# AdityaNG/SOccDPT

Measured on AMD Instinct MI355X. Metric: frames/sec SOccDPT_V3 swin2_tiny_256 @256px (depth+seg+points+occupancy forward), higher is better.
Workload: dtype mixed fp16 + f16x3 (SOCCDPT_PREC_MIXED: fp16 MFMA operands, x3 split per the shipped precision map; f32 accumulate)

## Files before the change

### soccdpt_amd/csrc/capi.cpp

```cpp
#include <hip/hip_runtime.h>

#include <cstring>
#include <cstdlib>
#include <string>

#include "internal.h"
#include "calibrate.h"
#include "train.h"
#include "kernels.h"
#include "occ_eval.h"
#include "visualise.h"
#include "occ_view.h"
#include "batch_targets.h"
#include "../../include/soccdpt_vis.h"
#include "../../include/soccdpt_occ_view.h"
#include "../../include/soccdpt_data.h"

using namespace soccdpt;

static std::string g_create_error;

namespace soccdpt {
LaunchTimer*& launch_timer() {
    static thread_local LaunchTimer* t = nullptr;
    return t;
}
unsigned long long& launch_counter() {
    static thread_local unsigned long long n = 0;
    return n;
}
void set_last_error(const std::string& msg) { g_create_error = msg; }
}

static double occ_cells(const soccdpt_config& c) { return (double)c.grid[0] * c.grid[1] * c.grid[2] * c.num_classes; }

static int fail(Handle* h, const std::string& msg) {
    if (h) h->err = msg; else g_create_error = msg;
    return 1;
}

static int profiled_project(Handle* h, const float* inv, const float* seg, int B, int in_h, int in_w, float* inv_up, float* seg_up, float* points,
                            uint32_t* occ_bits, int clear_bits, hipStream_t st) {
    const soccdpt_config& c = h->cfg;
    const double px = (double)c.cam_width * c.cam_height * B;
    const double bytes = (double)B * in_h * in_w * 4.0 * (1 + c.num_classes) + px * 4.0 * ((inv_up ? 1 : 0) + (seg_up ? c.num_classes : 0) + (points ? 3 : 0));
    ProfScope ps(h->prof, "project_voxelise", 0.0, bytes, st);
    return launch_project(c, inv, seg, B, in_h, in_w, inv_up, seg_up, points, occ_bits, clear_bits, st, h->err);
}
static int profiled_occ_expand(Handle* h, const uint32_t* bits, int B, float* occ, hipStream_t st) {
// ... 308 lines not shown
}

int soccdpt_occ_expand(void* handle, const uint32_t* dev_bits, int B, float* dev_occ, void* stream) {
    Handle* h = static_cast<Handle*>(handle);
    if (!h) return 1;
    if (B <= 0) return fail(h, "soccdpt_occ_expand: empty batch");
    return profiled_occ_expand(h, dev_bits, B, dev_occ, (hipStream_t)stream);
}

int soccdpt_occ_zero(void* handle, int B, float* dev_occ, void* stream) {
    Handle* h = static_cast<Handle*>(handle);
    if (!h) return 1;
    if (B <= 0 || !dev_occ) return fail(h, "soccdpt_occ_zero: bad argument");
    ProfScope ps(h->prof, "occ_zero", 0.0, occ_cells(h->cfg) * 4.0 * B, (hipStream_t)stream);
    return launch_occ_zero(h->cfg, B, dev_occ, (hipStream_t)stream, h->err);
}

int soccdpt_occ_set(void* handle, const uint32_t* dev_bits, int B, float* dev_occ, void* stream) {
    Handle* h = static_cast<Handle*>(handle);
    if (!h) return 1;
    if (B <= 0 || !dev_occ || !dev_bits) return fail(h, "soccdpt_occ_set: bad argument");
    ProfScope ps(h->prof, "occ_set", 0.0, occ_cells(h->cfg) * 0.125, (hipStream_t)stream);
    return launch_occ_set(h->cfg, dev_bits, B, dev_occ, (hipStream_t)stream, h->err);
}

int soccdpt_forward(void* handle, const float* dev_x, int B, float* dev_inv_up, float* dev_seg_up, float* dev_points,
                    float* dev_occ, uint32_t* dev_occ_bits, void* dev_workspace, size_t workspace_bytes, void* stream) {
    Handle* h = static_cast<Handle*>(handle);
    if (!h) return 1;
    if (B <= 0) return fail(h, "soccdpt_forward: empty batch");
    const int S = h->img;
    hipStream_t st = (hipStream_t)stream;
    float *inv, *seg;
    int rc = network_at_head(h, "soccdpt_forward", dev_x, B, dev_workspace, workspace_bytes, st, &inv, &seg);
    if (rc) return rc;
    const bool occ_on = h->cfg.compute_occ != 0;
    if (occ_on && !dev_occ_bits) return fail(h, "soccdpt_forward: compute_occ needs dev_occ_bits");
    rc = profiled_project(h, inv, seg, B, S, S, dev_inv_up, dev_seg_up, dev_points, occ_on ? dev_occ_bits : nullptr, 1, st);
    if (rc) return rc;
    if (occ_on && dev_occ) rc = profiled_occ_expand(h, dev_occ_bits, B, dev_occ, st);
    return rc;
}

int soccdpt_voxelise_frames(void* handle, const float* dev_inv_up, const float* dev_seg, int B, int in_h, int in_w, uint32_t* dev_frame_bits,
                            int clear_bits, void* stream) {
    Handle* h = static_cast<Handle*>(handle);
    if (!h) return 1;
    if (!dev_inv_up || !dev_seg || !dev_frame_bits) return fail(h, "soccdpt_voxelise_frames: null argument");
    if (B <= 0 || in_h <= 0 || in_w <= 0) return fail(h, "soccdpt_voxelise_frames: empty input");
    return profiled_voxelise_frames(h, dev_inv_up, dev_seg, B, in_h, in_w, dev_frame_bits, clear_bits, (hipStream_t)stream);
}

int soccdpt_occ_expand_frames(void* handle, const uint32_t* dev_frame_bits, int B, float* dev_occ, void* stream) {
    Handle* h = static_cast<Handle*>(handle);
    if (!h) return 1;
    if (!dev_frame_bits || !dev_occ) return fail(h, "soccdpt_occ_expand_frames: null argument");
    if (B <= 0) return fail(h, "soccdpt_occ_expand_frames: empty batch");
    return profiled_occ_expand_frames(h, dev_frame_bits, B, dev_occ, (hipStream_t)stream);
}

int soccdpt_forward_frames(void* handle, const float* dev_x, int B, float* dev_inv_up, float* dev_seg_up, float* dev_points, float* dev_occ,
                           uint32_t* dev_occ_bits, uint32_t* dev_frame_bits, void* dev_workspace, size_t workspace_bytes, void* stream) {
    Handle* h = static_cast<Handle*>(handle);
    if (!h) return 1;
    if (B <= 0) return fail(h, "soccdpt_forward_frames: empty batch");
    if (!dev_x || !dev_workspace) return fail(h, "soccdpt_forward_frames: null argument");
    if (!h->cfg.compute_occ) return fail(h, "soccdpt_forward_frames: the handle was created without compute_occ");
    if (!dev_inv_up) return fail(h, "soccdpt_forward_frames: dev_inv_up is required (the per-frame voxelisation reads the inverse depth back)");
    if (!dev_frame_bits) return fail(h, "soccdpt_forward_frames: dev_frame_bits is required");
    const int S = h->img;
    hipStream_t st = (hipStream_t)stream;
// ... 271 lines not shown
    if (d.x3 && d.tune == 12 && d.splitk <= 1 && !d.ln_g &&
        (d.stride != 1 || d.pad != 1 || d.in_halo != 1 || d.Hi || d.Wi || d.gather1 || d.grp_rows || d.seg2_k || d.stamps))
        return fail(nullptr, "soccdpt_op_igemm: x3 configuration 12 has no generalised addressing");
    if (launch_igemm(d, (hipStream_t)stream, err)) return fail(nullptr, err);
    if (a->gn_stats && a->gn_count && (gn_bm <= 0 || a->gn_hw % gn_bm))
        return fail(nullptr, "soccdpt_op_igemm: statistics requested but the chosen tile has no statistics epilogue (tune forces a tile without one)");
    if (a->gn_stats && a->gn_count && launch_gn_finish(a->gn_part, a->gn_stats, a->M / a->gn_hw, a->gn_hw / gn_bm, a->N / a->gn_cpg, a->gn_hw, a->gn_cpg, 1e-5f, (hipStream_t)stream, err))
        return fail(nullptr, err);
    return 0;
}

int soccdpt_op_depth_tail(const void* dev_d1, const void* dev_wt, const float* dev_bias, const float* dev_w4, float b4, float* dev_out, int precision,
                          int B, int h, int w, void* stream) {
    std::string err;
    if (!dev_d1 || !dev_wt || !dev_bias || !dev_w4 || !dev_out) return fail(nullptr, "soccdpt_op_depth_tail: null argument");
    if (precision != SOCCDPT_PREC_BF16 && precision != SOCCDPT_PREC_F16) return fail(nullptr, "soccdpt_op_depth_tail: precision is SOCCDPT_PREC_BF16 or _F16");
    if (B <= 0 || h <= 0 || w <= 0) return fail(nullptr, "soccdpt_op_depth_tail: B, h, w must be positive");
    if ((2 * h) % 8 || (2 * w) % 16) return fail(nullptr, "soccdpt_op_depth_tail: the output (2h x 2w) must be a multiple of 8 x 16");
    if (launch_depth_tail(static_cast<const bf16_t*>(dev_d1), static_cast<const bf16_t*>(dev_wt), dev_bias, dev_w4, b4, dev_out, precision == SOCCDPT_PREC_F16 ? 1 : 0,
                          B, h, w, (hipStream_t)stream, err))
        return fail(nullptr, err);
    return 0;
}

int soccdpt_op_seg_tail(const float* dev_part, int nplanes, const float* dev_bias, float* dev_tmp, float* dev_out, int B, int h, int w, int sigmoid,
                        void* stream) {
    std::string err;
    if (!dev_part || !dev_bias || !dev_tmp || !dev_out) return fail(nullptr, "soccdpt_op_seg_tail: null argument");
    if (nplanes < 1 || B <= 0 || h <= 0 || w <= 0) return fail(nullptr, "soccdpt_op_seg_tail: nplanes, B, h and w must be positive");
    if (launch_seg_tail_parts(dev_part, nplanes, dev_bias, dev_tmp, dev_out, B, h, w, sigmoid ? 1 : 0, (hipStream_t)stream, err)) return fail(nullptr, err);
    return 0;
}

int soccdpt_op_wgrad_tn(const void* dev_a, long lda, const void* dev_b, long ldb, size_t K, int Nout, int C, int taps, int rp, int precision, float* dev_scratch,
                        size_t scratch_floats, float* dev_out, void* stream) {
    std::string err;
    if (!dev_a || !dev_b || !dev_scratch || !dev_out) return fail(nullptr, "soccdpt_op_wgrad_tn: null argument");
    if (precision != SOCCDPT_PREC_BF16 && precision != SOCCDPT_PREC_F16 && precision != SOCCDPT_PREC_F16X3) return fail(nullptr, "soccdpt_op_wgrad_tn: bf16, fp16 or f16x3 operands");
    const OpFmt fmt = precision == SOCCDPT_PREC_F16X3 ? OpFmt::X3 : (precision == SOCCDPT_PREC_F16 ? OpFmt::F16 : OpFmt::BF16);
    if (tr_wgrad_tn(dev_a, lda, dev_b, ldb, K, Nout, C, taps, rp, fmt, dev_scratch, scratch_floats, dev_out,
                    (hipStream_t)stream, err))
        return fail(nullptr, err);
    return 0;
}

size_t soccdpt_op_train_layer_bwd_scratch_bytes(const soccdpt_train_layer_bwd_args* args) {
    std::string err;
    const size_t n = args ? train_layer_bwd_scratch_bytes(*args, err) : 0;
    if (!n) fail(nullptr, args ? err : "soccdpt_op_train_layer_bwd_scratch_bytes: null args");
    return n;
}
int soccdpt_op_train_layer_bwd(void* handle, const soccdpt_train_layer_bwd_args* args, void* dev_scratch, size_t scratch_bytes, uint32_t* path_out, void* stream) {
    Handle* h = static_cast<Handle*>(handle);
    if (!h) return fail(nullptr, "soccdpt_op_train_layer_bwd: null handle");
    if (!args) return fail(h, "soccdpt_op_train_layer_bwd: null args");
    unsigned path = 0;
    if (train_layer_bwd(*h, *args, dev_scratch, scratch_bytes, &path, (hipStream_t)stream, h->err)) return 1;
    if (path_out) *path_out = path;
    return 0;
}

size_t soccdpt_op_train_aux_scratch_bytes(const soccdpt_train_aux_args* args) {
    std::string err;
    const size_t n = args ? train_aux_scratch_bytes(*args, err) : 0;
    if (!n) fail(nullptr, args ? err : "soccdpt_op_train_aux_scratch_bytes: null args");
    return n;
// ... 302 lines not shown
```

### soccdpt_amd/csrc/elementwise.hip

```cpp
#include <type_traits>

#include "half16.h"
#include "kernels.h"
#include "ln_body.h"

namespace soccdpt {

__device__ __forceinline__ float row_sum(float v) {
    auto ror = [](float x, auto n) {
        return __builtin_bit_cast(float, __builtin_amdgcn_update_dpp(0, __builtin_bit_cast(int, x), 0x120 + decltype(n)::value, 0xf, 0xf, true));
    };
    v += ror(v, std::integral_constant<int, 8>{});
    v += ror(v, std::integral_constant<int, 4>{});
    v += ror(v, std::integral_constant<int, 2>{});
    v += ror(v, std::integral_constant<int, 1>{});
    return v;
}

#define LAUNCH_HF(hf, K, ...)                                   \
    do {                                                        \
        if (hf) SOCCDPT_LAUNCH((K<true>), __VA_ARGS__);     \
        else SOCCDPT_LAUNCH((K<false>), __VA_ARGS__);       \
    } while (0)

// ... 428 lines not shown
    for (size_t i = (size_t)blockIdx.x * blockDim.x + threadIdx.x; i < total; i += (size_t)gridDim.x * blockDim.x) {
        const int ox = (int)(i % W);
        size_t r = i / W;
        const int oy = (int)(r % H), b = (int)(r / H);
        const float fy = sy * (float)oy, fx = sx * (float)ox;
        const int y0 = (int)fy, x0 = (int)fx;
        const int y1 = y0 + (y0 < h - 1), x1 = x0 + (x0 < w - 1);
        const float ly = fy - (float)y0, lx = fx - (float)x0, hy = 1.f - ly, hx = 1.f - lx;
        const float* base = in + (size_t)b * h * w * 3;
#pragma unroll
        for (int c = 0; c < 3; ++c) {
            const float v = hy * (hx * base[((size_t)y0 * w + x0) * 3 + c] + lx * base[((size_t)y0 * w + x1) * 3 + c]) +
                            ly * (hx * base[((size_t)y1 * w + x0) * 3 + c] + lx * base[((size_t)y1 * w + x1) * 3 + c]);
            const float a = sigmoid ? 1.f / (1.f + expf(-v)) : 0.5f * tanhf(v) + 0.5f;
            out[((size_t)(b * 3 + c) * H + oy) * W + ox] = a;
        }
    }
}

__global__ __launch_bounds__(256) void seg_logits_finish_kernel(const float* __restrict__ part , const float* __restrict__ bias, float* __restrict__ out ,
                                                                 size_t M, int T) {
    for (size_t m = (size_t)blockIdx.x * blockDim.x + threadIdx.x; m < M; m += (size_t)gridDim.x * blockDim.x) {
        float4 a = *reinterpret_cast<const float4*>(part + m * 4);
        for (int t = 1; t < T; ++t) {
            const float4 v = *reinterpret_cast<const float4*>(part + ((size_t)t * M + m) * 4);
            a.x += v.x; a.y += v.y; a.z += v.z;
        }
        out[m * 3 + 0] = a.x + bias[0];
        out[m * 3 + 1] = a.y + bias[1];
        out[m * 3 + 2] = a.z + bias[2];
    }
}

int launch_seg_tail_parts(const float* part, int ntiles, const float* bias, float* tmp, float* seg, int B, int h, int wd, int sigmoid, hipStream_t st, std::string& err) {
    const size_t M = (size_t)B * h * wd;
    size_t blocks = (M + 255) / 256;
    if (blocks > 2048) blocks = 2048;
    SOCCDPT_LAUNCH(seg_logits_finish_kernel, dim3((unsigned)blocks), dim3(256), 0, st, part, bias, tmp, M, ntiles);
    if (check_launch("seg_logits_finish", err)) return 1;
    const size_t total = (size_t)B * 4 * h * wd;
    blocks = (total + 255) / 256;
    if (blocks > 2048) blocks = 2048;
    SOCCDPT_LAUNCH(seg_up_act_kernel, dim3((unsigned)blocks), dim3(256), 0, st, tmp, seg, B, h, wd, sigmoid);
    return check_launch("seg_up_act", err);
}

int launch_seg_tail(const void* feat, int feat_is_f32, int hf, const float* w, const float* bias, float* tmp, float* seg, int B, int h, int wd,
                    int sigmoid, hipStream_t st, std::string& err, int* path) {
    if (!ptr_aligned16(feat) || (!feat_is_f32 && !ptr_aligned16(w))) { err = "seg_tail: 16-byte aligned features (and weights beside 16-bit features)"; return 1; }
    if (path) *path = feat_is_f32 ? SOCCDPT_FWD_PATH_SEG_F32 : SOCCDPT_FWD_PATH_SEG_16;
    const int M = B * h * wd;
    const dim3 grid((unsigned)(((size_t)M * 16 + 255) / 256));
    unsigned gl = grid.x > 2048 ? 2048 : grid.x;
    if (feat_is_f32) SOCCDPT_LAUNCH(conv1x1_c3_f32_kernel, grid, dim3(256), 0, st, static_cast<const float*>(feat), w, bias, tmp, M);
    else LAUNCH_HF(hf, conv1x1_c3_kernel, dim3(gl), dim3(256), 0, st, static_cast<const bf16_t*>(feat), w, bias, tmp, M);
    if (check_launch("conv1x1_c3", err)) return 1;
    const size_t total = (size_t)B * 4 * h * wd;
    size_t blocks = (total + 255) / 256;
    if (blocks > 2048) blocks = 2048;
    SOCCDPT_LAUNCH(seg_up_act_kernel, dim3((unsigned)blocks), dim3(256), 0, st, tmp, seg, B, h, wd, sigmoid);
    return check_launch("seg_up_act", err);
}

template <bool F16>
__global__ void cvt_bf16_kernel(const float* __restrict__ in, bf16_t* __restrict__ out, size_t n) {
    for (size_t i = (size_t)blockIdx.x * blockDim.x + threadIdx.x; i < n; i += (size_t)gridDim.x * blockDim.x) out[i] = f2h<F16>(in[i]);
}
// ... 144 lines not shown
```

### soccdpt_amd/csrc/internal.h

```cpp
#pragma once
#include <hip/hip_runtime.h>
#include <stdint.h>

#include <memory>
#include <string>
#include <unordered_map>
#include <vector>

#include "../../include/soccdpt_hip.h"
#include "launch.h"
#include "params.h"

namespace soccdpt {

struct Prepared;

struct ProfRec {
    const char* name;
    double flops, bytes;
    size_t first_pair, n_pairs;
};
struct Profiler : LaunchTimer {
    bool on = false;
    std::vector<ProfRec> recs;
// ... 30 lines not shown
    }
};

struct SiteRec {
    int M, N, K, taps, cfg, count;
    char name[16];
};

struct Handle {
    soccdpt_config cfg;
    int device = 0;
    int img = 256;
    Arch arch;
    std::string err;
    bool prof_sites = false;
    std::vector<SiteRec> sites;
    std::unordered_map<long long, int> tune_by_shape;
    bool fuse_qkv = true;
    int fuse_qkv_mask = 3;
    int mlp_fuse_max = 128;
    std::unordered_map<std::string, int> prec_map;
    int prec_source = -1;
    unsigned long long calib_fp = 0;
    bool calib_fp_valid = false;
    std::vector<WeightSlot> weights;
    ModelP params;
    const float* W(PRef r) const { return r.i < 0 ? nullptr : weights[r.i].ptr; }
    float* G(PRef r) const { return r.i < 0 ? nullptr : weights[r.i].grad; }
    std::unordered_map<std::string, int> index;
    size_t prepared_bytes = 0;
    Prepared* prep = nullptr;
    bool is_prepared = false;
    int launches = 0;
    Profiler prof;
    int n_streams = 1;
    std::vector<hipStream_t> sub_streams;
    std::vector<hipEvent_t> join_events;
    bool use_graph = false;
    struct GraphKey {
        const void *x = nullptr, *inv = nullptr, *seg = nullptr, *ws = nullptr;
        int B = 0, streams = 0;
        bool operator==(const GraphKey& o) const { return x == o.x && inv == o.inv && seg == o.seg && ws == o.ws && B == o.B && streams == o.streams; }
    } graph_key;
    struct WsKey {
        const void* ws = nullptr;
        int B = 0, streams = 0;
        bool operator==(const WsKey& o) const { return ws == o.ws && B == o.B && streams == o.streams; }
    } ws_key;
    int ws_zero_fills = 0;
    struct TrainKey {
        const void* ws = nullptr;
        int B = 0;
        float dropout_p = 0.f;
        int amp = 0;
        float drop_path = 0.f;
    } train_key;
    float train_drop_path = 0.f;
    std::shared_ptr<void> layer_state;
    int train_amp = 0;
    hipGraph_t graph = nullptr;
    hipGraphExec_t graph_exec = nullptr;
    hipStream_t graph_stream = nullptr;
    hipEvent_t graph_in = nullptr, graph_out = nullptr;
    int eager_calls = 0;
    ~Handle();
};

int model_init(Handle& h, std::string& err);
int model_bind(Handle& h, const char* key, const void* ptr, const int64_t* shape, int ndim, std::string& err);
size_t model_workspace_bytes(Handle& h, int B);
int model_prepare(Handle& h, void* prepared, size_t bytes, hipStream_t stream, std::string& err);
int model_network(Handle& h, const float* x, int B, float* inv256, float* seg256, void* ws, size_t ws_bytes, hipStream_t stream,
                  std::string& err);

std::vector<std::string> model_prec_groups(const Handle& h);
void model_prec_default(Handle& h);
int model_prec_set(Handle& h, const char* pattern, int fmt, std::string& err);
bool model_prec_x2w_ok(const std::string& group);
int model_set_streams(Handle& h, int n, std::string& err);
void model_drop_graph(Handle& h);
int model_workspace_tensor(Handle& h, int B, const char* name, size_t* byte_offset, size_t* elems, int* kind, int* H, int* W, int* C);

int launch_project(const soccdpt_config& cfg, const float* inv, const float* seg, int B, int in_h, int in_w, float* inv_up,
                   float* seg_up, float* points, uint32_t* occ_bits, int clear_bits, hipStream_t stream, std::string& err);
int launch_occ_expand(const soccdpt_config& cfg, const uint32_t* bits, int B, float* occ, hipStream_t stream, std::string& err);
int launch_occ_zero(const soccdpt_config& cfg, int B, float* occ, hipStream_t stream, std::string& err);
int launch_occ_set(const soccdpt_config& cfg, const uint32_t* bits, int B, float* occ, hipStream_t stream, std::string& err);
int launch_occ_or(const soccdpt_config& cfg, uint32_t* dst, const uint32_t* src, int nsets, hipStream_t stream, std::string& err);

int launch_voxelise_frames(const soccdpt_config& cfg, const float* inv_up, const float* seg, int B, int in_h, int in_w, uint32_t* frame_bits,
                           int clear_bits, hipStream_t stream, std::string& err);
int launch_occ_expand_frames(const soccdpt_config& cfg, const uint32_t* frame_bits, int B, float* occ, hipStream_t stream, std::string& err);

}
```

### soccdpt_amd/csrc/kernels.h

```cpp
#pragma once
#include <hip/hip_runtime.h>
#include <stdint.h>

#include <string>

#include "../../include/soccdpt_hip.h"
#include "igemm.h"

namespace soccdpt {

inline int check_launch(const char* what, std::string& err) {
    hipError_t e = hipGetLastError();
    if (e != hipSuccess) {
        err = std::string(what) + ": " + hipGetErrorString(e);
        return 1;
    }
    return 0;
}

inline bool ptr_aligned16(const void* p) { return reinterpret_cast<uintptr_t>(p) % 16 == 0; }

int launch_patch_embed(const float* x, const float* w, const float* bias, const float* g, const float* beta, float* xf, bf16_t* xb,
                       int hf, int B, int S, int C0, hipStream_t st, std::string& err);
int launch_ln_residual(const float* y, const float* g, const float* beta, float* xf, bf16_t* xb, bf16_t* halo, float* halo_f32, int hf, int M,
                       int C, int residual, int res, int merge, hipStream_t st, std::string& err, const float* row_scale = nullptr, int rows_per_scale = 1,
                       int hf_halo = -1, int* path = nullptr);
int launch_merge_gather(const void* in, void* out, int B, int R, int C, int elem_bytes, hipStream_t st, std::string& err);
int launch_bilinear(const void* in, int in_is_bf16, float* out_f32, bf16_t* out_bf16, float* out_f32_halo, int out_halo, int hf, int B, int h,
                    int w, int H, int W, int C, hipStream_t st, std::string& err, int* path = nullptr);
int launch_seg_tail(const void* feat, int feat_is_f32, int hf, const float* w, const float* bias, float* tmp, float* seg, int B, int h, int wd,
                    int sigmoid, hipStream_t st, std::string& err, int* path = nullptr);
int launch_seg_tail_parts(const float* part, int ntiles, const float* bias, float* tmp, float* seg, int B, int h, int wd, int sigmoid, hipStream_t st, std::string& err);
inline int patch_w_ld(int C0) { return C0 <= 128 ? 128 : 192; }
int launch_patch_w(const float* w, float* out, int C0, hipStream_t st, std::string& err);
int launch_cvt_bf16(const float* in, bf16_t* out, size_t n, int hf, hipStream_t st, std::string& err);
int launch_conv_w(const float* in, const float* scale, void* out, int out_is_f32, int hf, int Cout, int Cin, hipStream_t st, std::string& err);
int launch_bn_fold(const float* g, const float* b, const float* mean, const float* var, float* scale, float* shift, int C, hipStream_t st,
                   std::string& err);
int launch_qkv_bias(const float* q, const float* v, float* out, int C, hipStream_t st, std::string& err);
int launch_logit_scale(const float* ls, float* out, int H, hipStream_t st, std::string& err);
int launch_cpb_table(const float* w0, const float* b0, const float* w2, float* table, int ws, int pws, int H, hipStream_t st,
                     std::string& err);

int launch_depth_tail(const bf16_t* d1, const bf16_t* wt, const float* bias, const float* w4, float b4, float* out, int hf, int B, int h,
                      int w, hipStream_t st, std::string& err);

size_t metrics_scratch_bytes(int B, int C);
int launch_depth_metrics(const float* pred, const float* gt, const uint8_t* mask, int B, size_t npix, float* out, void* scratch, hipStream_t st,
                         std::string& err);
int launch_iou_metrics(const float* pred, const float* gt, int B, int C, size_t npix, float* out, void* scratch, hipStream_t st, std::string& err);

size_t loss_scratch_bytes(int B, int H, int W, int h, int w);
int launch_training_loss(int B, int H, int W, int h, int w, int C, int compute_ss, float alpha, float w_d, float w_s, const float* inv,
                         const float* seg, const float* y_disp, const uint8_t* mask_disp, const float* y_seg, const uint8_t* mask_seg,
                         float* out, float* d_inv, float* d_seg, void* scratch, hipStream_t st, std::string& err);

int launch_gt_occupancy(int B, int H, int W, int C, const double* intr, const double* pc_scale, const double* pc_shift, const double* rot27,
                        const float* occ_shape, const int* grid, float threshold, const float* disparity, const int32_t* seg_class, float* depth,
                        double* points, uint32_t* counts, uint8_t* occ, hipStream_t st, std::string& err);

size_t upsample_bwd_scratch_bytes(const soccdpt_config& cfg, int B, int h);
int launch_upsample_bwd(const soccdpt_config& cfg, const float* inv_up, const float* d_inv_up, const float* d_seg_up, const float* d_points, int B, int h, int w,
                        float* d_inv, float* d_seg, void* scratch, hipStream_t st, std::string& err);

int launch_input_transform_u8(const uint8_t* img, int B, int Hs, int Ws, int Hd, int Wd, const double* mean, const double* stdv, float* out,
// ... 85 lines not shown
```

### soccdpt_amd/csrc/model.cpp

```cpp
#include <cstdio>
#include <cstdlib>
#include <cstring>

#include <unordered_set>

#include "internal.h"
#include "kernels.h"

namespace soccdpt {

struct BlockW {
    const void *qkv_w, *proj_w, *fc1_w, *fc2_w;
    float *qkv_bias, *scale, *table, *bias_acc;
};
struct RcuW { const void *w1, *w2; };
struct RnBlockW { const void *ds_w = nullptr, *c1_w = nullptr, *c2_w = nullptr, *c3_w = nullptr; };
struct VitBlockW { const void *qkv_w, *proj_w, *fc1_w, *fc2_w; };
struct HybridW {
    const void* stem_w = nullptr;
    std::vector<RnBlockW> rn;
    const void* pe_w = nullptr;
    float* pos = nullptr;
    std::vector<VitBlockW> blocks;
    const void *ro_w[2] = {nullptr, nullptr}, *pp_w[2] = {nullptr, nullptr}, *pp4_w = nullptr;
// ... 830 lines not shown
               RUN(launch_bilinear(w.oc[0], 0, nullptr, fH == 2 ? nullptr : static_cast<bf16_t*>(w.path1), fH == 2 ? static_cast<float*>(w.path1) : nullptr, 1, fH == 2 ? 0 : fH, B, r, r,
                                   2 * r, 2 * r, F, st, err)); }
    }
    const int r1 = 2 * a.fres(0), r0 = 4 * a.fres(0);
    {
        IgemmDesc d = conv(w.path1, F, P.d0_w, F / 2, r1);
        d.bias = W(MP.depth.c0.b);
        if (fD2 <= 1 && F == 256) {
            d.out_op = w.d1; d.out_fmt = MIX ? fD2 : -1;
            RUN(gemm(d, fH));
            PROF("depth_tail_fused", 2.0 * B * r0 * r0 * 32.0 * 9.0 * (F / 2), 0.0);
            RUN(launch_depth_tail(static_cast<const bf16_t*>(w.d1), static_cast<const bf16_t*>(P.d2_w), W(MP.depth.c2.b), W(MP.depth.c4.w), P.d4_b, inv256, fD2, B, r1, r1, st, err));
        } else {
            const bool d1_16 = fH <= 1 && !MIX;
            if (d1_16) d.out_op = w.d1; else to_plain(d, w.d1, fH);
            RUN(gemm(d, fH));
            { PROF("bilinear_resize", 0.0, (double)B * r1 * r1 * (F / 2) * (2.0 + 8.0));
              RUN(launch_bilinear(w.d1, d1_16 ? 1 : 0, nullptr, fD2 == 2 ? nullptr : static_cast<bf16_t*>(w.d1u), fD2 == 2 ? static_cast<float*>(w.d1u) : nullptr, 1, fD2 == 2 ? 0 : fD2, B, r1,
                                  r1, r0, r0, F / 2, st, err)); }
            d = conv(w.d1u, F / 2, P.d2_w, 32, r0);
            d.bias = W(MP.depth.c2.b); d.act = ACT_RELU; d.dot_w = W(MP.depth.c4.w); d.dot_b = P.d4_b; d.out_dot = inv256;
            RUN(gemm(d, fD2));
        }
        const int fS1 = MIX ? GF("head.s1") : fH;
        const bool s1_f32 = fS1 >= 2;
        d = conv(w.path1, F, P.s0_w, F, r1);
        d.bias = P.bn_shift; d.act = ACT_RELU;
        if (seg_dot3_active(h)) {
            d.dot3 = 1; d.dot_w = W(MP.seg.c4.w); d.out_dot = static_cast<float*>(w.s1);
            d.f16 = fH == 1;
            const int parts = F / igemm_dot3_bn(d);
            RUN(gemm(d, fH));
            PROF("seg_tail", 0.0, (double)B * r1 * r1 * (parts * 16.0 + 12.0 + 12.0 + 48.0));
            RUN(launch_seg_tail_parts(static_cast<const float*>(w.s1), parts, W(MP.seg.c4.b), w.s2, seg256, B, r1, r1, h.cfg.sigmoid, st, err));
        } else {
        if (s1_f32) to_plain(d, w.s1, fH); else { d.out_op = w.s1; d.out_fmt = MIX ? 1 : -1; }
        RUN(gemm(d, fH));
        { PROF("seg_tail", 0.0, (double)B * r1 * r1 * (F * 2.0 + 12.0 + 48.0));
          RUN(launch_seg_tail(w.s1, s1_f32 ? 1 : 0, fS1 == 1, W(MP.seg.c4.w), W(MP.seg.c4.b), w.s2, seg256, B, r1, r1, h.cfg.sigmoid, st, err)); }
        }
        ++launches;
    }
#undef RUN
#undef PROF
    return 0;
}

static void chunk_range(int B, int n, int i, int& lo, int& hi) {
    const int base = B / n, rem = B % n;
    lo = i * base + (i < rem ? i : rem);
    hi = lo + base + (i < rem ? 1 : 0);
}

static int n_chunks(const Handle& h, int B) {
    int n = h.n_streams < 1 ? 1 : h.n_streams;
    return n > B ? B : n;
}

static void carve_all(const Handle& h, int B, Arena& ar, std::vector<Workspace>& ws) {
    ar.take<float>((size_t)B * h.img * h.img * (1 + h.cfg.num_classes));
    const int n = n_chunks(h, B);
    ws.resize(n);
    for (int i = 0; i < n; ++i) {
        int lo, hi;
        chunk_range(B, n, i, lo, hi);
        carve(h, hi - lo, ar, ws[i]);
    }
}

size_t model_workspace_bytes(Handle& h, int B) {
    Arena ar(nullptr, 0);
    std::vector<Workspace> ws;
    carve_all(h, B, ar, ws);
    return ar.off + 256;
}

int model_set_streams(Handle& h, int n, std::string& err) {
    if (n < 1 || n > 8) { err = "soccdpt_set_streams: n must be in 1..8"; return 1; }
    while ((int)h.sub_streams.size() < n - 1) {
        hipStream_t s;
        if (hipStreamCreateWithFlags(&s, hipStreamNonBlocking) != hipSuccess) { err = "soccdpt_set_streams: stream creation failed"; return 1; }
        h.sub_streams.push_back(s);
    }
    while ((int)h.join_events.size() < n) {
        hipEvent_t e;
        if (hipEventCreateWithFlags(&e, hipEventDisableTiming) != hipSuccess) { err = "soccdpt_set_streams: event creation failed"; return 1; }
        h.join_events.push_back(e);
    }
    h.n_streams = n;
    model_drop_graph(h);
    return 0;
}

static int network_eager(Handle& h, const float* x, int B, float* inv256, float* seg256, void* ws, size_t ws_bytes, hipStream_t st,
                         std::string& err) {
    Arena ar(ws, ws_bytes);
    std::vector<Workspace> wsp;
    carve_all(h, B, ar, wsp);
    if (ar.off > ws_bytes) { err = "soccdpt_network: workspace too small"; return 1; }
    const int n = (int)wsp.size();
// ... 23 lines not shown
    }
    h.launches = launches;
    return 0;
}

void model_drop_graph(Handle& h) {
    if (h.graph_exec) (void)hipGraphExecDestroy(h.graph_exec);
    if (h.graph) (void)hipGraphDestroy(h.graph);
    h.graph_exec = nullptr;
    h.graph = nullptr;
    h.eager_calls = 0;
}

int model_network(Handle& h, const float* x, int B, float* inv256, float* seg256, void* ws, size_t ws_bytes, hipStream_t st,
                  std::string& err) {
    if (!h.is_prepared) { err = "soccdpt_network: call soccdpt_prepare after binding weights"; return 1; }
    if (B <= 0 || !x || !inv256 || !seg256 || !ws) { err = "soccdpt_network: bad argument"; return 1; }
    {
        int dev = -1;
        (void)hipGetDevice(&dev);
        if (dev != h.device) { err = "soccdpt_network: the handle was created on device " + std::to_string(h.device) + " but device " + std::to_string(dev) + " is current"; return 1; }
        const size_t need = model_workspace_bytes(h, B);
        if (ws_bytes < need) { err = "soccdpt_network: workspace too small (soccdpt_workspace_bytes)"; return 1; }
        Handle::WsKey wk{ws, B, h.n_streams};
        if (!(wk == h.ws_key)) {
            model_drop_graph(h);
            if (hipMemsetAsync(ws, 0, need, st) != hipSuccess) { err = "soccdpt_network: workspace zero-fill failed"; return 1; }
            h.ws_key = wk;
            h.ws_zero_fills++;
        }
    }
    if (!h.use_graph || h.prof.on) return network_eager(h, x, B, inv256, seg256, ws, ws_bytes, st, err);
    Handle::GraphKey key;
    key.x = x; key.inv = inv256; key.seg = seg256; key.ws = ws; key.B = B; key.streams = h.n_streams;
    if (!(key == h.graph_key)) {
        model_drop_graph(h);
        h.graph_key = key;
    }
    if (h.eager_calls++ == 0 && !h.graph_exec) return network_eager(h, x, B, inv256, seg256, ws, ws_bytes, st, err);
    hipStream_t cs = h.graph_stream;
    if (hipEventRecord(h.graph_in, st) != hipSuccess || hipStreamWaitEvent(cs, h.graph_in, 0) != hipSuccess) {
        err = "soccdpt_network: graph fork failed";
        return 1;
    }
    if (!h.graph_exec) {
        if (hipStreamBeginCapture(cs, hipStreamCaptureModeThreadLocal) != hipSuccess) { err = "soccdpt_network: begin capture failed"; return 1; }
        const int rc = network_eager(h, x, B, inv256, seg256, ws, ws_bytes, cs, err);
        hipGraph_t g = nullptr;
        const hipError_t ec = hipStreamEndCapture(cs, &g);
        if (rc || ec != hipSuccess || !g) {
            if (g) (void)hipGraphDestroy(g);
            if (!rc) err = std::string("soccdpt_network: end capture failed: ") + hipGetErrorString(ec);
            return 1;
        }
        h.graph = g;
        if (hipGraphInstantiate(&h.graph_exec, g, nullptr, nullptr, 0) != hipSuccess) {
            model_drop_graph(h);
            err = "soccdpt_network: graph instantiate failed";
            return 1;
        }
    }
    if (hipGraphLaunch(h.graph_exec, cs) != hipSuccess) { err = "soccdpt_network: hipGraphLaunch failed"; return 1; }
    if (hipEventRecord(h.graph_out, cs) != hipSuccess || hipStreamWaitEvent(st, h.graph_out, 0) != hipSuccess) {
        err = "soccdpt_network: graph join failed";
        return 1;
    }
    return 0;
// ... 4 lines not shown
```

### soccdpt_amd/lib.py

```python
from __future__ import annotations

import ctypes
import os
from typing import Optional, Sequence

import numpy as np
import torch

_HERE = os.path.dirname(os.path.abspath(__file__))
LIB_PATH = os.environ.get("SOCCDPT_LIB_PATH") or os.path.join(_HERE, "libsoccdpt_hip.so")

ABI_VERSION = 12
BACKBONE_IDS = {"swin2t16_256": 0, "swin2b24_384": 1, "vitb_rn50_384": 2, "swin2l24_384": 3, "swinl12_384": 5}
PREC_BF16 = 0
PREC_F32 = 1
PREC_F16 = 2
PREC_F16X3 = 3
PREC_MIXED = 4
PREC_F16X2W = 5


class SoccdptConfig(ctypes.Structure):
    _fields_ = [
        ("abi_version", ctypes.c_int32),
# ... 258 lines not shown
        "soccdpt_pack_targets": (ci, [vp, ci, cs, vp, ci, vp, ci, vp, ci, ci, ci, ci, ci, vp, vp, vp, vp, vp]),
        "soccdpt_pack_expand": (ci, [vp, ci, cs, vp, ci, ci, ci, ci, vp, vp]),
    }


PACK_PROTOTYPES = _pack_prototypes()


def _swin1_prototypes() -> dict:
    vp, ci, cf = ctypes.c_void_p, ctypes.c_int, ctypes.c_float
    return {
        "soccdpt_swin1_window_attention": (ci, [vp, vp, vp, vp, ci, ci, ci, ci, ci, ci, ci, vp]),
        "soccdpt_swin1_ln_rows": (ci, [vp, vp, vp, vp, ci, ci, ci, cf, vp]),
        "soccdpt_swin1_merge_ln": (ci, [vp, vp, vp, vp, ci, ci, ci, ci, cf, vp]),
    }


SWIN1_PROTOTYPES = _swin1_prototypes()


def _occ_view_prototypes() -> dict:
    vp, ci, cs, cd = ctypes.c_void_p, ctypes.c_int, ctypes.c_size_t, ctypes.c_double
    i32, u8, f64 = ctypes.POINTER(ctypes.c_int32), ctypes.POINTER(ctypes.c_uint8), ctypes.POINTER(cd)
    return {
        "soccdpt_occ_view_columns": (ci, [vp, ci, i32, ci, ci, ci, vp, vp, vp, vp, vp]),
        "soccdpt_occ_view_paint": (ci, [vp, vp, ci, ci, ci, ci, ci, vp, ci, u8, ci, ci, ci, ci, ci, vp, cs, cs, cs, cs, vp]),
        "soccdpt_occ_view_iou2d": (ci, [vp, ci, vp, ci, cs, ci, vp, vp]),
        "soccdpt_occ_view_splat": (ci, [vp, ci, i32, ci, f64, f64, cd, ci, cd, ci, ci, vp, vp]),
        "soccdpt_occ_view_resolve": (ci, [vp, vp, ci, ci, ci, ci, ci, vp, ci, vp, cs, cs, cs, cs, vp]),
    }


OCC_VIEW_PROTOTYPES = _occ_view_prototypes()
PACK_INDEX_BITS = (1, 2, 4, 8)


def load_library() -> ctypes.CDLL:
    global _lib
    if _lib is not None:
        return _lib
    if not os.path.exists(LIB_PATH):
        raise RuntimeError(
            f"{LIB_PATH} is missing: build it with `python -c 'import __graft_entry__ as g; g.build()'` "
            "(make -C soccdpt_amd/csrc).  The SOccDPT MI355X path has no CPU fallback.")
    L = ctypes.CDLL(LIB_PATH)
    for table in (PROTOTYPES, VIS_PROTOTYPES, DATA_PROTOTYPES, PACK_PROTOTYPES, SWIN1_PROTOTYPES, OCC_VIEW_PROTOTYPES):
        for symbol, (restype, argtypes) in table.items():
            fn = getattr(L, symbol)
            fn.restype, fn.argtypes = restype, argtypes
    if L.soccdpt_abi_version() != ABI_VERSION:
        raise RuntimeError("libsoccdpt_hip.so ABI version mismatch; rebuild the library")
    for which, cls in ((0, SoccdptConfig), (1, IgemmArgs), (2, KernelStat), (3, CalibReport), (4, CalibOptions), (5, TrainLayerBwdArgs), (6, TrainAuxArgs), (7, FwdAuxArgs)):
        if L.soccdpt_sizeof(which) != ctypes.sizeof(cls):
            raise RuntimeError(f"libsoccdpt_hip.so: sizeof mismatch for {cls.__name__}: library {L.soccdpt_sizeof(which)}, binding {ctypes.sizeof(cls)}")
    _lib = L
    return L


def _ptr(t: Optional[torch.Tensor]) -> Optional[int]:
    if t is None:
        return None
    assert t.is_contiguous(), "device tensors handed to libsoccdpt_hip must be contiguous"
    return t.data_ptr()


def _stream_ptr(device: torch.device) -> int:
    return torch.cuda.current_stream(device).cuda_stream


def _call(symbol: str, *args, device: torch.device, guard: bool = True):
    L = load_library()
    fn = getattr(L, symbol)
    if guard:
        with torch.cuda.device(device):
            rc = fn(*args, _stream_ptr(device))
    else:
        rc = fn(*args, _stream_ptr(device))
    if rc != 0:
        raise RuntimeError(f"{symbol} failed: {L.soccdpt_last_error(None).decode()}")
# ... 352 lines not shown
def op_igemm(x, wt, M, N, Cin, taps=1, ldx=0, H=0, W=0, bias=None, res1=None, res2=None, act=0, out_f32=None,
             act_on_f32=0, out_bf16=None, out_halo=0, dot_w=None, dot_b=0.0, out_dot=None, tune=-1, f32=0, precision=None, splitk=1, sk_part=None, sk_count=None,
             conv=None, gather1=0, grp_rows=0, grp_off=0, grp_stride=0, seg2_k=0, seg2_off=0, gn_stats=None, gn_part=None, gn_count=None, gn_cpg=0, gn_hw=0,
             stamps=None, sk_defer=0, res2_h=0, res2_w=0, ln_g=None, ln_b=None, ln_xf=None, ln_halo=None, ln_residual=1, dot3=0, out_fmt=-1,
             halo_fmt=-1):
    c = conv or {}
    a = IgemmArgs(_ptr(x), _ptr(wt), M, N, Cin, taps, ldx, H, W, _ptr(bias), _ptr(res1), _ptr(res2), act, _ptr(out_f32),
                  act_on_f32, _ptr(out_bf16), out_halo, _ptr(dot_w), float(dot_b), _ptr(out_dot), tune,
                  int(precision) if precision is not None else (PREC_F32 if f32 else PREC_BF16), int(splitk), _ptr(sk_part), _ptr(sk_count),
                  0 if sk_part is None else sk_part.numel(), 0 if sk_count is None else sk_count.numel(),
                  1 if conv else 0, c.get("stride", 1), c.get("pad", 1), c.get("in_halo", 1), c.get("Hi", 0), c.get("Wi", 0), int(gather1),
                  int(grp_rows), int(grp_off), int(seg2_k), int(seg2_off), int(grp_stride),
                  _ptr(gn_stats), _ptr(gn_part), _ptr(gn_count), int(gn_cpg), int(gn_hw),
                  0 if gn_part is None else gn_part.numel(), 0 if gn_count is None else gn_count.numel(), _ptr(stamps), int(sk_defer),
                  int(res2_h), int(res2_w), _ptr(ln_g), _ptr(ln_b), _ptr(ln_xf), _ptr(ln_halo), int(ln_residual), int(dot3), int(out_fmt),
                  int(halo_fmt))
    _call("soccdpt_op_igemm", ctypes.byref(a), device=x.device, guard=False)


def op_depth_tail(d1, wt, bias, w4, b4, out, B, h, w, precision=PREC_BF16):
    _call("soccdpt_op_depth_tail", _ptr(d1), _ptr(wt), _ptr(bias), _ptr(w4), float(b4), _ptr(out), int(precision), int(B), int(h), int(w),
          device=d1.device, guard=False)


def op_seg_tail(part, nplanes, bias, tmp, out, B, h, w, sigmoid):
    _call("soccdpt_op_seg_tail", _ptr(part), int(nplanes), _ptr(bias), _ptr(tmp), _ptr(out), int(B), int(h), int(w), 1 if sigmoid else 0,
          device=part.device, guard=False)


def op_gn_finish(part, stats, B, tps, groups, hw, cpg, eps=1e-5):
    _call("soccdpt_op_gn_finish", _ptr(part), _ptr(stats), int(B), int(tps), int(groups), int(hw), int(cpg), float(eps), device=part.device, guard=False)


def op_gn_apply(raw, stats, gamma, beta, hw, w, cpg, part=None, tps=0, raw2=None, stats2=None, part2=None, tps2=0, gamma2=None, beta2=None, res=None,
                out_f32=None, out_op=None, out_halo=None, out_format=PREC_F32, relu=True, eps=1e-5):
    M, C = raw.shape
    _call("soccdpt_op_gn_apply", _ptr(raw), _ptr(stats), _ptr(part), int(tps), _ptr(gamma), _ptr(beta), _ptr(raw2), _ptr(stats2), _ptr(part2), int(tps2),
          _ptr(gamma2), _ptr(beta2), _ptr(res), _ptr(out_f32), _ptr(out_op), _ptr(out_halo), int(out_format), 1 if relu else 0, M, int(hw),
          int(w), int(C), int(cpg), float(eps), device=raw.device, guard=False)


def op_vit_attention(qkv, out, B, N, heads, precision=PREC_BF16, out_x3=False):
    if out_x3:
        _call("soccdpt_op_vit_attention_out", _ptr(qkv), _ptr(out), int(precision), 1, B, N, heads, device=qkv.device, guard=False)
    else:
        _call("soccdpt_op_vit_attention", _ptr(qkv), _ptr(out), int(precision), B, N, heads, device=qkv.device, guard=False)


def op_input_transform_u8(frames: torch.Tensor, Hd: int, Wd: int, mean=(0.5, 0.5, 0.5), std=(0.5, 0.5, 0.5)) -> torch.Tensor:
    assert frames.dtype == torch.uint8 and frames.dim() == 4 and frames.shape[3] == 3 and frames.is_cuda
    B, Hs, Ws, _ = frames.shape
    out = torch.empty((B, 3, Hd, Wd), dtype=torch.float32, device=frames.device)
    m, s = (ctypes.c_double * 3)(*mean), (ctypes.c_double * 3)(*std)
    _call("soccdpt_input_transform_u8", _ptr(frames), B, Hs, Ws, Hd, Wd, m, s, _ptr(out), device=frames.device)
    return out


_DATA_DTYPES = {torch.uint8: DATA_U8, torch.uint16: DATA_U16, torch.float32: DATA_F32}


def op_data_targets(seg: torch.Tensor, colors: torch.Tensor, disp: Optional[torch.Tensor] = None, flip: bool = False, want_onehot: bool = True,
                    want_class_map: bool = False, want_y_disp: Optional[bool] = None, want_unmatched: bool = True) -> dict:
    assert seg.is_cuda and seg.dtype == torch.uint8 and seg.dim() == 4 and seg.shape[3] == 3, "seg must be a cuda uint8 [B,H,W,3] tensor"
    assert colors.is_cuda and colors.dtype == torch.uint8 and colors.dim() == 2 and colors.shape[1] == 3, "colors must be a cuda uint8 [C,3] tensor"
    B, H, W, _ = seg.shape
    C = colors.shape[0]
# ... 174 lines not shown
```

Before: 3957.

## Fuse seg tail logits and upsample into one kernel and fold occupancy-bit clearing

Replaces the two-launch segmentation tail (logit reduction, then bilinear upsample plus activation) with a single fused kernel. The upsample recomputes the partial-logit sums per output pixel instead of reading them back from a temporary. The same kernel also zeroes the occupancy bit buffer, so the later projection step skips its own clear, removing a memset/launch. The fused path recomputes each logit four times per output pixel, and there is no grid-wide sync between writing the logits temp and the upsample reading it, but the upsample only recomputes and never reads the temp.

Measured after the change: 3973 (median of 6 runs). No clear change (+0.4%).

```diff
diff --git a/include/soccdpt_fwd_ends.h b/include/soccdpt_fwd_ends.h
--- /dev/null
+++ b/include/soccdpt_fwd_ends.h
@@ -0,0 +1,18 @@
+#ifndef SOCCDPT_FWD_ENDS_H
+#define SOCCDPT_FWD_ENDS_H
+
+#include <stddef.h>
+#include <stdint.h>
+
+#ifdef __cplusplus
+extern "C" {
+#endif
+
+int soccdpt_op_seg_tail_clear(const float* dev_part, int nplanes, const float* dev_bias, float* dev_tmp, float* dev_out, int B, int h, int w,
+                              int sigmoid, uint32_t* dev_zero, size_t nzero, void* stream);
+
+#ifdef __cplusplus
+}
+#endif
+
+#endif
diff --git a/soccdpt_amd/csrc/capi.cpp b/soccdpt_amd/csrc/capi.cpp
--- a/soccdpt_amd/csrc/capi.cpp
+++ b/soccdpt_amd/csrc/capi.cpp
@@ -15,6 +15,7 @@
 #include "../../include/soccdpt_vis.h"
 #include "../../include/soccdpt_occ_view.h"
 #include "../../include/soccdpt_data.h"
+#include "../../include/soccdpt_fwd_ends.h"
 
 using namespace soccdpt;
 
@@ -389,11 +390,16 @@
     const int S = h->img;
     hipStream_t st = (hipStream_t)stream;
     float *inv, *seg;
-    int rc = network_at_head(h, "soccdpt_forward", dev_x, B, dev_workspace, workspace_bytes, st, &inv, &seg);
-    if (rc) return rc;
     const bool occ_on = h->cfg.compute_occ != 0;
     if (occ_on && !dev_occ_bits) return fail(h, "soccdpt_forward: compute_occ needs dev_occ_bits");
-    rc = profiled_project(h, inv, seg, B, S, S, dev_inv_up, dev_seg_up, dev_points, occ_on ? dev_occ_bits : nullptr, 1, st);
+    const bool fold = occ_on && ptr_aligned16(dev_occ_bits) && model_fold_clear_ok(*h, B);
+    h->fold_bits = fold ? dev_occ_bits : nullptr;
+    h->fold_words = fold ? soccdpt_occ_words(h) : 0;
+    int rc = network_at_head(h, "soccdpt_forward", dev_x, B, dev_workspace, workspace_bytes, st, &inv, &seg);
+    h->fold_bits = nullptr;
+    h->fold_words = 0;
+    if (rc) return rc;
+    rc = profiled_project(h, inv, seg, B, S, S, dev_inv_up, dev_seg_up, dev_points, occ_on ? dev_occ_bits : nullptr, fold ? 0 : 1, st);
     if (rc) return rc;
     if (occ_on && dev_occ) rc = profiled_occ_expand(h, dev_occ_bits, B, dev_occ, st);
     return rc;
@@ -731,6 +737,16 @@
     return 0;
 }
 
+int soccdpt_op_seg_tail_clear(const float* dev_part, int nplanes, const float* dev_bias, float* dev_tmp, float* dev_out, int B, int h, int w, int sigmoid,
+                              uint32_t* dev_zero, size_t nzero, void* stream) {
+    std::string err;
+    if (!dev_part || !dev_bias || !dev_tmp || !dev_out) return fail(nullptr, "soccdpt_op_seg_tail_clear: null argument");
+    if (nplanes < 1 || B <= 0 || h <= 0 || w <= 0) return fail(nullptr, "soccdpt_op_seg_tail_clear: nplanes, B, h and w must be positive");
+    if (launch_seg_tail_parts(dev_part, nplanes, dev_bias, dev_tmp, dev_out, B, h, w, sigmoid ? 1 : 0, (hipStream_t)stream, err, dev_zero, dev_zero ? nzero : 0))
+        return fail(nullptr, "soccdpt_op_seg_tail_clear: " + err);
+    return 0;
+}
+
 int soccdpt_op_wgrad_tn(const void* dev_a, long lda, const void* dev_b, long ldb, size_t K, int Nout, int C, int taps, int rp, int precision, float* dev_scratch,
                         size_t scratch_floats, float* dev_out, void* stream) {
     std::string err;
diff --git a/soccdpt_amd/csrc/elementwise.hip b/soccdpt_amd/csrc/elementwise.hip
--- a/soccdpt_amd/csrc/elementwise.hip
+++ b/soccdpt_amd/csrc/elementwise.hip
@@ -484,7 +484,70 @@
     }
 }
 
-int launch_seg_tail_parts(const float* part, int ntiles, const float* bias, float* tmp, float* seg, int B, int h, int wd, int sigmoid, hipStream_t st, std::string& err) {
+__global__ __launch_bounds__(256) void seg_tail_fused_kernel(const float* __restrict__ part , const float* __restrict__ bias,
+                                                              float* __restrict__ logits , float* __restrict__ out , int B,
+                                                              int h, int w, int T, int sigmoid, uint32_t* __restrict__ zero, size_t nzero) {
+    const int H = 2 * h, W = 2 * w;
+    const size_t total = (size_t)B * H * W, M = (size_t)B * h * w;
+    const float sy = (float)(h - 1) / (float)(H - 1), sx = (float)(w - 1) / (float)(W - 1);
+    const float bs[3] = {bias[0], bias[1], bias[2]};
+    if (zero) {
+        const size_t n4 = nzero / 4;
+        uint4* z4 = reinterpret_cast<uint4*>(zero);
+        for (size_t i = (size_t)blockIdx.x * blockDim.x + threadIdx.x; i < n4; i += (size_t)gridDim.x * blockDim.x) z4[i] = uint4{0u, 0u, 0u, 0u};
+        for (size_t i = n4 * 4 + (size_t)blockIdx.x * blockDim.x + threadIdx.x; i < nzero; i += (size_t)gridDim.x * blockDim.x) zero[i] = 0u;
+    }
+    auto logit = [&](size_t m, float (&v)[3]) {
+        float4 a = *reinterpret_cast<const float4*>(part + m * 4);
+        for (int t = 1; t < T; ++t) {
+            const float4 p = *reinterpret_cast<const float4*>(part + ((size_t)t * M + m) * 4);
+            a.x += p.x; a.y += p.y; a.z += p.z;
+        }
+        v[0] = a.x + bs[0]; v[1] = a.y + bs[1]; v[2] = a.z + bs[2];
+    };
+    for (size_t m = (size_t)blockIdx.x * blockDim.x + threadIdx.x; m < M; m += (size_t)gridDim.x * blockDim.x) {
+        float v[3];
+        logit(m, v);
+        logits[m * 3 + 0] = v[0]; logits[m * 3 + 1] = v[1]; logits[m * 3 + 2] = v[2];
+    }
+    for (size_t i = (size_t)blockIdx.x * blockDim.x + threadIdx.x; i < total; i += (size_t)gridDim.x * blockDim.x) {
+        const int ox = (int)(i % W);
+        size_t r = i / W;
+        const int oy = (int)(r % H), b = (int)(r / H);
+        const float fy = sy * (float)oy, fx = sx * (float)ox;
+        const int y0 = (int)fy, x0 = (int)fx;
+        const int y1 = y0 + (y0 < h - 1), x1 = x0 + (x0 < w - 1);
+        const float ly = fy - (float)y0, lx = fx - (float)x0, hy = 1.f - ly, hx = 1.f - lx;
+        const size_t base = (size_t)b * h * w;
+        float v00[3], v01[3], v10[3], v11[3];
+        logit(base + (size_t)y0 * w + x0, v00); logit(base + (size_t)y0 * w + x1, v01);
+        logit(base + (size_t)y1 * w + x0, v10); logit(base + (size_t)y1 * w + x1, v11);
+#pragma unroll
+        for (int c = 0; c < 3; ++c) {
+            const float v = hy * (hx * v00[c] + lx * v01[c]) + ly * (hx * v10[c] + lx * v11[c]);
+            const float a = sigmoid ? 1.f / (1.f + expf(-v)) : 0.5f * tanhf(v) + 0.5f;
+            out[((size_t)(b * 3 + c) * H + oy) * W + ox] = a;
+        }
+    }
+}
+
+static bool seg_tail_two_launches() {
+    static const bool two = getenv("SOCCDPT_SEG_TAIL_FUSED") && atoi(getenv("SOCCDPT_SEG_TAIL_FUSED")) == 0;
+    return two;
+}
+int seg_tail_parts_launches() { return seg_tail_two_launches() ? 2 : 1; }
+
+int launch_seg_tail_parts(const float* part, int ntiles, const float* bias, float* tmp, float* seg, int B, int h, int wd, int sigmoid, hipStream_t st, std::string& err,
+                          uint32_t* zero, size_t nzero) {
+    if (!seg_tail_two_launches()) {
+        if (!ptr_aligned16(part) || !ptr_aligned16(zero)) { err = "seg_tail: 16-byte aligned partial logits (and words to clear)"; return 1; }
+        const size_t total = (size_t)B * 4 * h * wd;
+        size_t blocks = (total + 255) / 256;
+        if (blocks > 2048) blocks = 2048;
+        SOCCDPT_LAUNCH(seg_tail_fused_kernel, dim3((unsigned)blocks), dim3(256), 0, st, part, bias, tmp, seg, B, h, wd, ntiles, sigmoid, zero, nzero);
+        return check_launch("seg_tail_fused", err);
+    }
+    if (zero && hipMemsetAsync(zero, 0, nzero * sizeof(uint32_t), st) != hipSuccess) { err = "seg_tail: clearing failed"; return 1; }
     const size_t M = (size_t)B * h * wd;
     size_t blocks = (M + 255) / 256;
     if (blocks > 2048) blocks = 2048;
diff --git a/soccdpt_amd/csrc/internal.h b/soccdpt_amd/csrc/internal.h
--- a/soccdpt_amd/csrc/internal.h
+++ b/soccdpt_amd/csrc/internal.h
@@ -86,15 +86,17 @@
     Prepared* prep = nullptr;
     bool is_prepared = false;
     int launches = 0;
+    uint32_t* fold_bits = nullptr;
+    size_t fold_words = 0;
     Profiler prof;
     int n_streams = 1;
     std::vector<hipStream_t> sub_streams;
     std::vector<hipEvent_t> join_events;
     bool use_graph = false;
     struct GraphKey {
-        const void *x = nullptr, *inv = nullptr, *seg = nullptr, *ws = nullptr;
+        const void *x = nullptr, *inv = nullptr, *seg = nullptr, *ws = nullptr, *bits = nullptr;
         int B = 0, streams = 0;
-        bool operator==(const GraphKey& o) const { return x == o.x && inv == o.inv && seg == o.seg && ws == o.ws && B == o.B && streams == o.streams; }
+        bool operator==(const GraphKey& o) const { return x == o.x && inv == o.inv && seg == o.seg && ws == o.ws && bits == o.bits && B == o.B && streams == o.streams; }
     } graph_key;
     struct WsKey {
         const void* ws = nullptr;
@@ -131,6 +133,7 @@
 void model_prec_default(Handle& h);
 int model_prec_set(Handle& h, const char* pattern, int fmt, std::string& err);
 bool model_prec_x2w_ok(const std::string& group);
+bool model_fold_clear_ok(const Handle& h, int B);
 int model_set_streams(Handle& h, int n, std::string& err);
 void model_drop_graph(Handle& h);
 int model_workspace_tensor(Handle& h, int B, const char* name, size_t* byte_offset, size_t* elems, int* kind, int* H, int* W, int* C);
diff --git a/soccdpt_amd/csrc/kernels.h b/soccdpt_amd/csrc/kernels.h
--- a/soccdpt_amd/csrc/kernels.h
+++ b/soccdpt_amd/csrc/kernels.h
@@ -30,7 +30,9 @@
                     int w, int H, int W, int C, hipStream_t st, std::string& err, int* path = nullptr);
 int launch_seg_tail(const void* feat, int feat_is_f32, int hf, const float* w, const float* bias, float* tmp, float* seg, int B, int h, int wd,
                     int sigmoid, hipStream_t st, std::string& err, int* path = nullptr);
-int launch_seg_tail_parts(const float* part, int ntiles, const float* bias, float* tmp, float* seg, int B, int h, int wd, int sigmoid, hipStream_t st, std::string& err);
+int launch_seg_tail_parts(const float* part, int ntiles, const float* bias, float* tmp, float* seg, int B, int h, int wd, int sigmoid, hipStream_t st, std::string& err,
+                          uint32_t* zero = nullptr, size_t nzero = 0);
+int seg_tail_parts_launches();
 inline int patch_w_ld(int C0) { return C0 <= 128 ? 128 : 192; }
 int launch_patch_w(const float* w, float* out, int C0, hipStream_t st, std::string& err);
 int launch_cvt_bf16(const float* in, bf16_t* out, size_t n, int hf, hipStream_t st, std::string& err);
diff --git a/soccdpt_amd/csrc/model.cpp b/soccdpt_amd/csrc/model.cpp
--- a/soccdpt_amd/csrc/model.cpp
+++ b/soccdpt_amd/csrc/model.cpp
@@ -886,7 +886,9 @@
             const int parts = F / igemm_dot3_bn(d);
             RUN(gemm(d, fH));
             PROF("seg_tail", 0.0, (double)B * r1 * r1 * (parts * 16.0 + 12.0 + 12.0 + 48.0));
-            RUN(launch_seg_tail_parts(static_cast<const float*>(w.s1), parts, W(MP.seg.c4.b), w.s2, seg256, B, r1, r1, h.cfg.sigmoid, st, err));
+            RUN(launch_seg_tail_parts(static_cast<const float*>(w.s1), parts, W(MP.seg.c4.b), w.s2, seg256, B, r1, r1, h.cfg.sigmoid, st, err, h.fold_bits,
+                                      h.fold_bits ? h.fold_words : 0));
+            launches += seg_tail_parts_launches() - 2;
         } else {
         if (s1_f32) to_plain(d, w.s1, fH); else { d.out_op = w.s1; d.out_fmt = MIX ? 1 : -1; }
         RUN(gemm(d, fH));
@@ -920,6 +922,11 @@
         chunk_range(B, n, i, lo, hi);
         carve(h, hi - lo, ar, ws[i]);
     }
+}
+
+bool model_fold_clear_ok(const Handle& h, int B) {
+    static const bool off = getenv("SOCCDPT_FOLD_CLEAR") && atoi(getenv("SOCCDPT_FOLD_CLEAR")) == 0;
+    return !off && n_chunks(h, B) == 1 && seg_dot3_active(h);
 }
 
 size_t model_workspace_bytes(Handle& h, int B) {
@@ -1009,7 +1016,7 @@
     }
     if (!h.use_graph || h.prof.on) return network_eager(h, x, B, inv256, seg256, ws, ws_bytes, st, err);
     Handle::GraphKey key;
-    key.x = x; key.inv = inv256; key.seg = seg256; key.ws = ws; key.B = B; key.streams = h.n_streams;
+    key.x = x; key.inv = inv256; key.seg = seg256; key.ws = ws; key.bits = h.fold_bits; key.B = B; key.streams = h.n_streams;
     if (!(key == h.graph_key)) {
         model_drop_graph(h);
         h.graph_key = key;
diff --git a/soccdpt_amd/lib.py b/soccdpt_amd/lib.py
--- a/soccdpt_amd/lib.py
+++ b/soccdpt_amd/lib.py
@@ -314,6 +314,16 @@
 
 
 OCC_VIEW_PROTOTYPES = _occ_view_prototypes()
+
+
+def _fwd_ends_prototypes() -> dict:
+    vp, ci, cs = ctypes.c_void_p, ctypes.c_int, ctypes.c_size_t
+    return {
+        "soccdpt_op_seg_tail_clear": (ci, [vp, ci, vp, vp, vp, ci, ci, ci, ci, vp, cs, vp]),
+    }
+
+
+FWD_ENDS_PROTOTYPES = _fwd_ends_prototypes()
 PACK_INDEX_BITS = (1, 2, 4, 8)
 
 
@@ -326,7 +336,7 @@
             f"{LIB_PATH} is missing: build it with `python -c 'import __graft_entry__ as g; g.build()'` "
             "(make -C soccdpt_amd/csrc).  The SOccDPT MI355X path has no CPU fallback.")
     L = ctypes.CDLL(LIB_PATH)
-    for table in (PROTOTYPES, VIS_PROTOTYPES, DATA_PROTOTYPES, PACK_PROTOTYPES, SWIN1_PROTOTYPES, OCC_VIEW_PROTOTYPES):
+    for table in (PROTOTYPES, VIS_PROTOTYPES, DATA_PROTOTYPES, PACK_PROTOTYPES, SWIN1_PROTOTYPES, OCC_VIEW_PROTOTYPES, FWD_ENDS_PROTOTYPES):
         for symbol, (restype, argtypes) in table.items():
             fn = getattr(L, symbol)
             fn.restype, fn.argtypes = restype, argtypes
@@ -745,6 +755,11 @@
     _call("soccdpt_op_gn_finish", _ptr(part), _ptr(stats), int(B), int(tps), int(groups), int(hw), int(cpg), float(eps), device=part.device, guard=False)
 
 
+def op_seg_tail_clear(part, nplanes, bias, tmp, out, B, h, w, sigmoid, zero=None, nzero=0):
+    _call("soccdpt_op_seg_tail_clear", _ptr(part), int(nplanes), _ptr(bias), _ptr(tmp), _ptr(out), int(B), int(h), int(w), 1 if sigmoid else 0,
+          _ptr(zero), int(nzero), device=part.device, guard=False)
+
+
 def op_gn_apply(raw, stats, gamma, beta, hw, w, cpg, part=None, tps=0, raw2=None, stats2=None, part2=None, tps2=0, gamma2=None, beta2=None, res=None,
                 out_f32=None, out_op=None, out_halo=None, out_format=PREC_F32, relu=True, eps=1e-5):
     M, C = raw.shape
```
